# TobiaMarcucci/warm-start-hybrid-mpc

Hardware: AMD Instinct MI355X
Metric: QP subproblems/sec, cart-pole-with-walls N=20 synthetic frontier (higher is better)
Workload: dtype f64

## Files before the change

warm-start-hybrid-mpc_amd/csrc/hmpc_kernel.hip:

```cpp
#include <hip/hip_runtime.h>
#include <math.h>
#include <stdint.h>
#include <type_traits>

#include "hmpc_device.h"

#define WAVE 64
#define HMPC_REFINE_FROM_IT 12
#define HMPC_POLISH_RHO 1e5
#define HMPC_POLISH_RHO2 1e7
#define HMPC_POLISH_DELTA 1e-10
#define HMPC_RHO_OF(level) ((level) == 1 ? HMPC_POLISH_RHO2 : HMPC_POLISH_RHO)
#define HMPC_POLISH_ITERS 5
#define HMPC_POLISH_ROUNDS 6
#define HMPC_POLISH_ROUNDS_LAST 10
#define HMPC_ESC_MAX 2
#define HMPC_ESC_ITERS 6
#define HMPC_ESC_ENABLED(D) true
#define HMPC_LAM0_ROW 1
#ifndef HMPC_STABLE_DEN
#define HMPC_STABLE_DEN 1
#endif
#ifndef HMPC_PAIR
#define HMPC_PAIR 1
#endif
#ifndef HMPC_NARROW_PANEL
#define HMPC_NARROW_PANEL 1
#endif
#define HMPC_POLISH_ATTEMPTS 3
#define HMPC_RETRY (-1)
#define HMPC_POLISH_ROUNDS_WARM 3
#ifndef HMPC_POLISH_ROUNDS_OWN
#define HMPC_POLISH_ROUNDS_OWN 8
#endif
#define HMPC_POLISH_WARM_BMOVE 0.5
#define HMPC_POLISH_WARM_VMAX 1e-2
#ifndef HMPC_KERNEL_ATTR
#define HMPC_KERNEL_ATTR
#endif
#define DEV __device__ __forceinline__
#ifdef HMPC_NO_FENCE
#define HMPC_FENCE() do { } while (0)
#else
#define HMPC_FENCE() __builtin_amdgcn_sched_barrier(0)
#endif

#ifdef HMPC_STAMPS
#define DBG_SKIP(bit) (p.dbg & (1 << (bit)))
#define STAMP(k) do { long long now_ = clock64(); tacc[k] += now_ - tlast; tlast = clock64(); } while (0)
#define FSTAMP(k) do { long long now_ = clock64(); facc[k] += now_ - flast; flast = clock64(); } while (0)
#define FSTAMP_DECL long long flast = clock64()
static __device__ long long facc_dump[16];
#define FSTAMP_ARGS , long long *facc
#define FSTAMP_PASS , facc
#else
#define DBG_SKIP(bit) false
#define STAMP(k) do { } while (0)
#define FSTAMP(k) do { } while (0)
#define FSTAMP_DECL do { } while (0)
#define FSTAMP_ARGS
#define FSTAMP_PASS
#endif

DEV void lds_barrier()
{
    asm volatile("s_waitcnt lgkmcnt(0)\n\ts_barrier" ::: "memory");
}

DEV double wave_sum(double v)
{
#pragma unroll
    for (int o = 32; o > 0; o >>= 1) v += __shfl_xor(v, o);
    return v;
}
DEV double wave_max(double v)
{
#pragma unroll
    for (int o = 32; o > 0; o >>= 1) v = fmax(v, __shfl_xor(v, o));
    return v;
}
DEV double wave_min(double v)
{
#pragma unroll
    for (int o = 32; o > 0; o >>= 1) v = fmin(v, __shfl_xor(v, o));
    return v;
}

template <class D, int N>
DEV void block_reduce(double (&v)[N], const int (&op)[N], __attribute__((address_space(3))) double *red, int tid)
{
#pragma unroll
    for (int i = 0; i < N; i++) v[i] = op[i] == 0 ? wave_sum(v[i]) : op[i] == 1 ? wave_max(v[i]) : wave_min(v[i]);
    if constexpr (D::kNW > 1) {
        if ((tid & 63) == 0) {
#pragma unroll
            for (int i = 0; i < N; i++) red[(tid >> 6) * N + i] = v[i];
        }
        __syncthreads();
#pragma unroll
        for (int i = 0; i < N; i++) {
            double a = red[i];
#pragma unroll
            for (int w = 1; w < D::kNW; w++) {
                const double b = red[w * N + i];
                a = op[i] == 0 ? a + b : op[i] == 1 ? fmax(a, b) : fmin(a, b);
            }
            v[i] = a;
        }
        __syncthreads();
    }
}
template <class D> DEV double block_sum(double x, __attribute__((address_space(3))) double *red, int tid)
{
    double v[1] = {x};
    const int op[1] = {0};
    block_reduce<D, 1>(v, op, red, tid);
    return v[0];
}
template <class D> DEV double block_max(double x, __attribute__((address_space(3))) double *red, int tid)
{
    double v[1] = {x};
    const int op[1] = {1};
    block_reduce<D, 1>(v, op, red, tid);
    return v[0];
}
template <class D> DEV double block_min(double x, __attribute__((address_space(3))) double *red, int tid)
{
    double v[1] = {x};
    const int op[1] = {2};
    block_reduce<D, 1>(v, op, red, tid);
    return v[0];
}

DEV double bcast(double v, int src)
{
    const int lo = __builtin_amdgcn_readlane(__double2loint(v), src);
    const int hi = __builtin_amdgcn_readlane(__double2hiint(v), src);
    return __hiloint2double(hi, lo);
}

template <class D> DEV double bcast16(double v, int src)
{
    if constexpr (!D::kDpp) return bcast(v, src);
    const long x = __builtin_bit_cast(long, v);
    long r;
    switch (src) {
#define HMPC_DPP_CASE(n) case n: r = __builtin_amdgcn_update_dpp((long)0, x, 0x150 + n, 0xf, 0xf, false); break;
        HMPC_DPP_CASE(0) HMPC_DPP_CASE(1) HMPC_DPP_CASE(2) HMPC_DPP_CASE(3) HMPC_DPP_CASE(4) HMPC_DPP_CASE(5) HMPC_DPP_CASE(6) HMPC_DPP_CASE(7)
        HMPC_DPP_CASE(8) HMPC_DPP_CASE(9) HMPC_DPP_CASE(10) HMPC_DPP_CASE(11) HMPC_DPP_CASE(12) HMPC_DPP_CASE(13) HMPC_DPP_CASE(14)
#undef HMPC_DPP_CASE
    default: r = __builtin_amdgcn_update_dpp((long)0, x, 0x150 + 15, 0xf, 0xf, false); break;
    }
    return __builtin_bit_cast(double, r);
}

DEV double frcp(double b)
{
    double r = __builtin_amdgcn_rcp(b);
    r = fma(fma(-b, r, 1.0), r, r);
    r = fma(fma(-b, r, 1.0), r, r);
    return r;
}

typedef __attribute__((address_space(3))) double ldsd;
typedef __attribute__((address_space(3))) int ldsi;
typedef __attribute__((address_space(3))) unsigned char ldsb;

template <class IP, class DP>
struct Lists {
    IP rptr, rcol, cptr, crow, gptr, grow;
    DP rval, cval, gval, h;
};
typedef Lists<const ldsi *, const ldsd *> ListsL;
typedef Lists<const int *, const double *> ListsG;

struct Lds {
    ldsd *w, *lam, *nuf;
    ldsd *e;
    ldsd *Lm, *dinv, *Pr;
    ldsd *rd, *rdyn, *edyn, *g, *pv;
    ldsd *w1, *lam1, *nuf1, *w2, *lam2, *nuf2;
    ldsd *Mm, *PA, *q, *mv;
    ldsd *red;
    ldsi *flag;
    ldsd *x0;
    ldsi *fix;
    ldsd *AB, *P, *PT;
    ldsi *ei, *ej;
    ListsL L0;
    ListsG G0;
    double *LmG, *PrG;
    ldsd *Ls;
    ldsd *Lw;
    int abst, nup, lrows;
    const ldsd *Cdn, *sval;
    const ldsi *drow, *rinfo, *sptr, *srow, *nrow;
    const ldsd *ccv;
    const ldsb *cci;
    int term_on;
    unsigned long long fullfix;
};

template <int NX_, int NU_, int NUB_, int NW_, bool DPP_ = false>
struct Dims {
    static constexpr bool kDpp = DPP_;
    static constexpr int kNX = NX_, kNU = NU_, kNUB = NUB_;
    static constexpr int kNW = NW_, kNT = NW_ * 64;
    static constexpr bool kBig = NX_ < 0;
#ifdef HMPC_JIT_KC
    static constexpr int kKC = NX_ > 0 ? HMPC_JIT_KC : 0;
#else
    static constexpr int kKC = NX_ > 0 ? (NU_ == 7 ? 14 : 8) : 0;
#endif
    static DEV int nx(const DevProb &p) { return NX_ > 0 ? NX_ : p.nx; }
    static DEV int nu(const DevProb &p) { return NU_ > 0 ? NU_ : p.nu; }
    static DEV int nub(const DevProb &p) { return NU_ > 0 ? NUB_ : p.nub; }
    static DEV int nuc(const DevProb &p) { return NU_ > 0 ? NU_ - NUB_ : p.nuc; }
    static DEV int nz(const DevProb &p) { return NX_ > 0 ? NX_ + NU_ : p.nz; }
    static DEV int ne(const DevProb &p) { return NX_ > 0 ? (NX_ + NU_) * (NX_ + NU_ + 1) / 2 : p.ne; }
};

#define AB_STRIDE (D::kBig ? S.abst : nz)
template <class D> DEV decltype(auto) stage_lists(const Lds &S)
{
    if constexpr (D::kBig) return (S.G0);
    else return (S.L0);
}
template <class D> DEV auto fac_lm(const Lds &S)
{
    if constexpr (D::kBig) return S.LmG;
    else return S.Lm;
}
template <class D> DEV auto fac_pr(const Lds &S)
{
    if constexpr (D::kBig) return S.PrG;
    else return S.Pr;
}

template <int RS>
struct Rows {
    double s_[RS], zd_[RS], dz_[RS], prod_[RS];
    DEV double &s(int k, int) { return s_[k]; }
    DEV double &z(int k, int) { return zd_[k]; }
    DEV double &D(int k, int) { return zd_[k]; }
    DEV double &dz(int k, int) { return dz_[k]; }
    DEV double &prod(int k, int) { return prod_[k]; }
    DEV void bind(double *, int) {}
};
template <>
struct Rows<0> {
    double *__restrict__ s_, *__restrict__ zd_, *__restrict__ dz_, *__restrict__ prod_;
    DEV double &s(int, int r) { return s_[r]; }
    DEV double &z(int, int r) { return zd_[r]; }
    DEV double &D(int, int r) { return zd_[r]; }
    DEV double &dz(int, int r) { return dz_[r]; }
    DEV double &prod(int, int r) { return prod_[r]; }
    DEV void bind(double *base, int Mpad) { s_ = base; zd_ = base + Mpad; dz_ = base + 2 * Mpad; prod_ = base + 3 * Mpad; }
};
#define ROW_OPAQUE(r) asm volatile("" : "+v"(r))
#define LANE_OPAQUE(lane) asm volatile("" : "+v"(lane))
#ifdef HMPC_CHECK
#define HMPC_CHK(cond, bit) do { if (!(cond)) atomicOr(p.check_flag, 1u << (bit)); } while (0)
#else
#define HMPC_CHK(cond, bit) do { } while (0)
#endif
#define ROWS_BEGIN(k, rw)                                  \
    _Pragma("unroll") for (int k = 0; k < nslot; k++) {   \
        typename RM::Ref rw;                               \
        if (rm.at(p, k, lane, rw)) {                       \
            HMPC_CHK(rw.e >= 0 && rw.e < p.M, 0);
#define ROWS_END }}

DEV void row_decode(const DevProb &p, int r, int &t, int &lr)
{
    if (r >= p.Toff) {
        t = p.T - 1;
        lr = p.mreg + (r - p.Toff);
    } else {
        t = (int)__umulhi((unsigned)r, p.mreg_magic);
        lr = r - t * p.mreg;
    }
}

template <class D> DEV bool row_active(const DevProb &p, const ldsi *fix, int t, int lr, int term_on)
{
    const int nub = D::nub(p);
    if (lr >= p.mreg) return term_on;
    if (lr < p.nc) return true;
    int b = lr - p.nc;
    if (b >= nub) b -= nub;
    return fix[t * nub + b] < 0;
}

DEV int sym(int i, int l) { return i >= l ? i * (i + 1) / 2 + l : l * (l + 1) / 2 + i; }

template <class IP, class DP> DEV double list_dot(IP idx, DP val, int k0, int k1, const ldsd *v)
{
    double a0 = 0, a1 = 0, a2 = 0, a3 = 0;
    int k = k0;
    for (; k + 4 <= k1; k += 4) {
        const int i0 = idx[k], i1 = idx[k + 1], i2 = idx[k + 2], i3 = idx[k + 3];
        const double c0 = val[k], c1 = val[k + 1], c2 = val[k + 2], c3 = val[k + 3];
        a0 += c0 * v[i0];
        a1 += c1 * v[i1];
        a2 += c2 * v[i2];
        a3 += c3 * v[i3];
    }
    if (k + 2 <= k1) {
        const int i0 = idx[k], i1 = idx[k + 1];
        const double c0 = val[k], c1 = val[k + 1];
        a0 += c0 * v[i0];
        a1 += c1 * v[i1];
        k += 2;
    }
    if (k < k1) a2 += val[k] * v[idx[k]];
    return (a0 + a1) + (a2 + a3);
}
template <class L> DEV double row_dot(const L &st, int lr, const ldsd *v)
{
    return list_dot(st.rcol, st.rval, st.rptr[lr], st.rptr[lr + 1], v);
}
template <class L> DEV double col_dot(const L &st, int j, const ldsd *v)
{
    return list_dot(st.crow, st.cval, st.cptr[j], st.cptr[j + 1], v);
}
template <class L> DEV double gram(const L &st, int e, const ldsd *D)
{
    return list_dot(st.grow, st.gval, st.gptr[e], st.gptr[e + 1], D);
}
template <class D> DEV double crow_dot(const DevProb &p, const Lds &S, int lr, const ldsd *v)
{
    if constexpr (D::kBig) {
        if (S.Cdn && lr < p.mreg) {
            const int nz = D::nz(p);
            const int ri = S.rinfo[lr];
            if (ri >= 0) return S.sval[lr] * v[ri];
            const ldsd *c = S.Cdn + (-ri - 1) * nz;
            double a0 = 0, a1 = 0, a2 = 0, a3 = 0;
            int j = 0;
            for (; j + 4 <= nz; j += 4) {
                const double c0 = c[j], c1 = c[j + 1], c2 = c[j + 2], c3 = c[j + 3];
                const double v0 = v[j], v1 = v[j + 1], v2 = v[j + 2], v3 = v[j + 3];
                a0 += c0 * v0;
                a1 += c1 * v1;
                a2 += c2 * v2;
                a3 += c3 * v3;
            }
            for (; j < nz; j++) a0 += c[j] * v[j];
            return (a0 + a1) + (a2 + a3);
        }
    }
    if (lr < p.mreg) return row_dot(stage_lists<D>(S), lr, v);
    const int nz = D::nz(p);
    const double *c = p.Ct + (size_t)(lr - p.mreg) * nz;
    double a = 0;
    for (int j = 0; j < nz; j++) a += c[j] * v[j];
    return a;
}
template <class D> DEV double ccol_dot(const DevProb &p, const Lds &S, int t, int j, const ldsd *base)
{
    double a;
    if constexpr (D::kKC > 0) {
        const ldsd *eb = base + t * p.mreg, *cv = S.ccv + j * D::kKC;
        const ldsb *ci = S.cci + j * D::kKC;
        constexpr int H = D::kKC / 2;
        static_assert(D::kKC % 2 == 0, "padded columns come in two halves");
        double a0 = 0, a1 = 0;
#pragma unroll
        for (int hb = 0; hb < D::kKC; hb += H) {
            int idx[H];
            double cc[H], ee[H];
#pragma unroll
            for (int q = 0; q < H; q++) idx[q] = ci[hb + q];
#pragma unroll
            for (int q = 0; q < H; q++) cc[q] = cv[hb + q];
            HMPC_FENCE();
#pragma unroll
            for (int q = 0; q < H; q++) { HMPC_CHK(idx[q] >= 0 && idx[q] < p.mreg && j >= 0 && j < D::nz(p) && t >= 0 && t < p.T, 1); ee[q] = eb[idx[q]]; }
            HMPC_FENCE();
#pragma unroll
            for (int q = 0; q < H; q++) {
                if (q & 1) a1 += cc[q] * ee[q];
                else a0 += cc[q] * ee[q];
            }
        }
        a = a0 + a1;
    } else if (D::kBig && S.Cdn) {
        const int nz = D::nz(p);
        const ldsd *eb = base + t * p.mreg, *c = S.Cdn + j;
        double a0 = 0, a1 = 0;
        int r = 0;
        for (; r + 2 <= p.nd; r += 2) {
            a0 += c[r * nz] * eb[S.drow[r]];
            a1 += c[(r + 1) * nz] * eb[S.drow[r + 1]];
        }
        if (r < p.nd) a0 += c[r * nz] * eb[S.drow[r]];
        for (int k = S.sptr[j]; k < S.sptr[j + 1]; k++) {
            const int sr = S.srow[k];
            a1 += S.sval[sr] * eb[sr];
        }
        a = a0 + a1;
    } else {
        a = col_dot(stage_lists<D>(S), j, base + t * p.mreg);
    }
    if (S.term_on && t == p.T - 1) {
        if constexpr (D::kKC > 0) {
            a += S.mv[j];
        } else {
            const int nz = D::nz(p);
            const ldsd *vt = base + p.Toff;
            double a0 = 0, a1 = 0;
            int k = 0;
            for (; k + 2 <= p.nT; k += 2) {
                a0 += p.Ct[(size_t)k * nz + j] * vt[k];
                a1 += p.Ct[(size_t)(k + 1) * nz + j] * vt[k + 1];
            }
            if (k < p.nT) a0 += p.Ct[(size_t)k * nz + j] * vt[k];
            a += a0 + a1;
        }
    }
    return a;
}

template <class D, class RM> DEV void term_cols(const DevProb &p, const Lds &S, int lane, const ldsd *base)
{
    if constexpr (D::kKC > 0) {
        if (!S.term_on) return;
        constexpr int NZ = D::kNX + D::kNU, KT = RM::kSlots - RM::kSlotsFB;
        double acc[NZ];
#pragma unroll
        for (int j = 0; j < NZ; j++) acc[j] = 0.0;
#pragma unroll
        for (int k = 0; k < KT; k++) {
            const int row = k * D::kNT + lane;
            const bool ok = row < p.nT;
            const int rc = ok ? row : 0;
            const double v = ok ? base[p.Toff + rc] : 0.0;
            const double *c = p.Ct + (size_t)rc * NZ;
#pragma unroll
            for (int j = 0; j < NZ; j++) acc[j] += c[j] * v;
        }
        if constexpr (D::kNW == 1) {
#pragma unroll
            for (int j = 0; j < NZ; j++) acc[j] = wave_sum(acc[j]);
        } else {
            constexpr int CH = 40 / D::kNW;
#pragma unroll
            for (int j0 = 0; j0 < NZ; j0 += CH) {
                double v[CH];
                int op[CH];
#pragma unroll
                for (int q = 0; q < CH; q++) { v[q] = j0 + q < NZ ? acc[j0 + q] : 0.0; op[q] = 0; }
                block_reduce<D, CH>(v, op, S.red, lane);
#pragma unroll
// ... 1368 lines not shown
        for (int i = lane; i < nx; i += D::kNT) dw[i] = usex0 ? S.x0[i] : 0.0;
        __syncthreads();
    }
    for (int t = wave_sweeps ? T : 0; t < T; t++) {
        const auto Lm = fac_lm<D>(S) + t * lms;
        const ldsi *fx = S.fix + t * nub;
        const ldsd *x = dw + t * nz;
        for (int j = lane; j < nu; j += D::kNT) {
            double a = S.dinv[t * nu + j] * dw[t * nz + nx + j];
            const bool fixed = j >= nuc && fx[j - nuc] >= 0;
            if (!fixed)
                for (int l = 0; l < nx; l++) a += Lm[LM_X(nx, nu, l, j)] * x[l];
            S.mv[j] = a;
        }
        __syncthreads();
        for (int j = nu - 1; j >= 1; j--) {
            const double uj = S.mv[j];
            for (int i = lane; i < j; i += D::kNT) {
                const bool fixed = i >= nuc && fx[i - nuc] >= 0;
                if (!fixed) S.mv[i] -= Lm[LM_U(nx, nu, j, i)] * uj;
            }
            __syncthreads();
        }
        for (int i = lane; i < nu; i += D::kNT) dw[t * nz + nx + i] = -S.mv[i];
        __syncthreads();
        for (int i = lane; i < nx; i += D::kNT) {
            double a = csrc ? cs * csrc[t * nx + i] : 0.0;
            for (int l = 0; l < nz; l++) a += S.AB[i * AB_STRIDE + l] * dw[t * nz + l];
            dw[(t + 1) * nz + i] = a;
        }
        __syncthreads();
    }
    for (int o = lane; o < (T + 1) * nx; o += D::kNT) {
        const int t = o / nx, i = o - t * nx;
        double a = S.pv[o];
        const auto Pt = fac_pr<D>(S) + t * nxs;
        int l = 0;
        for (; l + 4 <= nx; l += 4) {
            const double p0 = Pt[sym(i, l)], p1 = Pt[sym(i, l + 1)], p2 = Pt[sym(i, l + 2)], p3 = Pt[sym(i, l + 3)];
            a += p0 * dw[t * nz + l] + p1 * dw[t * nz + l + 1] + p2 * dw[t * nz + l + 2] + p3 * dw[t * nz + l + 3];
        }
        for (; l < nx; l++) a += Pt[sym(i, l)] * dw[t * nz + l];
        dlam[o] = -a;
    }
    FSTAMP(8);
    {
        const int nslot = RS > 0 ? RS : p.Mpad / D::kNT;
        ROWS_BEGIN(k, rw)
            const double d = R.D(k, rw.e);
            if (d != 0.0)
                S.e[rw.e] = d * rm.dot(p, S, k, rw, dw) - S.e[rw.e];
        ROWS_END
    }
    __syncthreads();
    FSTAMP(9);
    const bool own_g = gsrc && gsrc != S.g;
    for (int o = lane; o < T * nub; o += D::kNT) {
        const int t = o / nub, b = o - t * nub;
        double a = 0;
        if (S.fix[o] >= 0) {
            const int c = nx + nuc + b;
            a = own_g ? gs * gsrc[t * nz + c] : 0.0;
            for (int j = 0; j < nz; j++) a -= S.P[c * nz + j] * dw[t * nz + j];
            a -= ccol_dot<D>(p, S, t, c, S.e);
            for (int l = 0; l < nx; l++) a += S.AB[l * AB_STRIDE + c] * dlam[(t + 1) * nx + l];
        }
        dnuf[o] = a;
    }
    for (int i = lane; i < nx; i += D::kNT) {
        double a = own_g ? gs * gsrc[i] : 0.0;
        for (int j = 0; j < nz; j++) a -= S.P[i * nz + j] * dw[j];
        a -= ccol_dot<D>(p, S, 0, i, S.e);
        for (int l = 0; l < nx; l++) a += S.AB[l * AB_STRIDE + i] * dlam[nx + l];
        dlam[i] = a;
    }
    __syncthreads();
    FSTAMP(10);
}

template <class D, int RS, class RM>
DEV void kkt_solve_reg(const DevProb &p, const Lds &S, Rows<RS> &R, const RM &rm, int lane, const ldsd *gsrc, double gs, bool usex0,
                       const ldsd *csrc, double cs, bool useb, ldsd *dw, ldsd *dlam, ldsd *dnuf FSTAMP_ARGS)
{
    constexpr int NX = D::kNX, NU = D::kNU, NUB = D::kNUB, NUC = NU - NUB, NZ = NX + NU;
    constexpr int NXS = NX * (NX + 1) / 2, LMS = LM_STAGE(NX, NU);
    const int T = p.T;
    FSTAMP_DECL;
    LANE_OPAQUE(lane);
    term_cols<D, RM>(p, S, lane, S.e);
    for (int o = lane; o < T * NZ; o += D::kNT) {
        const int t = o / NZ, j = o - t * NZ;
        const double a = (gsrc ? gs * gsrc[o] : 0.0) + ccol_dot<D>(p, S, t, j, S.e);
        S.g[o] = (useb ? S.g[o] : 0.0) - a;
    }
    for (int o = lane; o < T * NX; o += D::kNT) {
        const int t = o / NX, i = o - t * NX;
        double a = 0.0;
        if (csrc) {
#pragma unroll
            for (int l = 0; l < NX; l++) a += S.Pr[(t + 1) * NXS + sym(i, l)] * (cs * csrc[t * NX + l]);
        }
        S.pv[o] = a;
    }
    double pvr = 0.0;
    if (lane < NX) {
        pvr = -(gsrc ? gs * gsrc[T * NZ + lane] : 0.0);
        S.pv[T * NX + lane] = pvr;
    }
    __syncthreads();
    FSTAMP(6);
    LANE_OPAQUE(lane);
    if (D::kNW == 1 || lane < WAVE) {
        double ABcol[NX];
#pragma unroll
        for (int l = 0; l < NX; l++) ABcol[l] = lane < NZ ? S.AB[l * NZ + lane] : 0.0;
        const int rowoff = lane < NX ? lane * NU : lane < NZ ? LM_U(NX, NU, lane - NX, 0) : 0;
        const int rowlen = lane < NX ? NU : lane < NZ ? lane - NX : 0;
        const int gl = lane < NZ ? lane : 0, bl = (lane >= NX + NUC && lane < NZ) ? lane - NX - NUC : 0;
        const int pl = lane < NX ? lane : 0;
        double mrow_n[NU], mpre_n, qc_n;
        int f_n;
        {
            const ldsd *row = S.Lm + (T - 1) * LMS + rowoff;
#pragma unroll
            for (int j = 0; j < NU; j++) mrow_n[j] = row[j];
            mpre_n = S.g[(T - 1) * NZ + gl];
            f_n = S.fix[(T - 1) * NUB + bl];
            qc_n = S.pv[(T - 1) * NX + pl];
        }
        for (int t = T - 1; t >= 0; t--) {
            double mrow[NU];
#pragma unroll
            for (int j = 0; j < NU; j++) mrow[j] = j < rowlen ? mrow_n[j] : 0.0;
            const double mpre = lane < NZ ? mpre_n : 0.0;
            const int f = (lane >= NX + NUC && lane < NZ) ? f_n : -1;
            const double qv = pvr + qc_n;
            {
                const int tn = t > 0 ? t - 1 : 0;
                const ldsd *row = S.Lm + tn * LMS + rowoff;
#pragma unroll
                for (int j = 0; j < NU; j++) mrow_n[j] = row[j];
                mpre_n = S.g[tn * NZ + gl];
                f_n = S.fix[tn * NUB + bl];
                qc_n = S.pv[tn * NX + pl];
            }
            double v = mpre;
#pragma unroll
            for (int l = 0; l < NX; l++) v += ABcol[l] * bcast16<D>(qv, l);
            if (f >= 0) v = (useb && f == 1) ? -1.0 : 0.0;
#pragma unroll
            for (int j = 0; j < NUC; j++) v -= mrow[j] * bcast16<D>(v, NX + j);
            if (!((S.fullfix >> t) & 1ull)) {
#pragma unroll
                for (int j = NUC; j < NU; j++) v -= mrow[j] * bcast16<D>(v, NX + j);
            }
            if (lane >= NX && lane < NZ) dw[t * NZ + lane] = v;
            pvr = v;
            if (lane < NX) S.pv[t * NX + lane] = v;
        }
    }
    __syncthreads();
    FSTAMP(7);
    LANE_OPAQUE(lane);
    if (D::kNW == 1 || lane < WAVE) {
        double ABrow[NZ];
#pragma unroll
        for (int l = 0; l < NZ; l++) ABrow[l] = lane < NX ? S.AB[lane * NZ + l] : 0.0;
        double xr = (lane < NX && usex0) ? S.x0[lane] : 0.0;
        const int cl = lane < NU ? lane : 0, pl = lane < NX ? lane : 0;
        double lx_n[NX], lcol_n[NU], dinv_n, y_n, cdy_n;
        {
            const ldsd *colp = S.Lm + cl;
#pragma unroll
            for (int l = 0; l < NX; l++) lx_n[l] = colp[LM_X(NX, NU, l, 0)];
#pragma unroll
            for (int i = 1; i < NU; i++) lcol_n[i] = colp[LM_U(NX, NU, i, 0)];
            dinv_n = S.dinv[cl];
            y_n = dw[NX + cl];
            cdy_n = csrc ? csrc[pl] : 0.0;
        }
        for (int t = 0; t < T; t++) {
            double lx[NX], lcol[NU];
#pragma unroll
            for (int l = 0; l < NX; l++) lx[l] = lane < NU ? lx_n[l] : 0.0;
            lcol[0] = 0.0;
#pragma unroll
            for (int i = 1; i < NU; i++) lcol[i] = lane < i ? lcol_n[i] : 0.0;
            double cur = lane < NU ? dinv_n * y_n : 0.0;
            double xn = (csrc && lane < NX) ? cs * cdy_n : 0.0;
            {
                const int tn = t + 1 < T ? t + 1 : t;
                const ldsd *colp = S.Lm + tn * LMS + cl;
#pragma unroll
                for (int l = 0; l < NX; l++) lx_n[l] = colp[LM_X(NX, NU, l, 0)];
#pragma unroll
                for (int i = 1; i < NU; i++) lcol_n[i] = colp[LM_U(NX, NU, i, 0)];
                dinv_n = S.dinv[tn * NU + cl];
                y_n = dw[tn * NZ + NX + cl];
                cdy_n = csrc ? csrc[tn * NX + pl] : 0.0;
            }
#pragma unroll
            for (int l = 0; l < NX; l++) {
                const double xl = bcast16<D>(xr, l);
                cur += lx[l] * xl;
                xn += ABrow[l] * xl;
            }
#pragma unroll
            for (int j = NU - 1; j >= 0; j--) {
                const double uj = bcast16<D>(cur, j);
                cur -= lcol[j] * uj;
                xn -= ABrow[NX + j] * uj;
            }
            if (lane < NX) dw[t * NZ + lane] = xr;
            if (lane < NU) dw[t * NZ + NX + lane] = -cur;
            xr = xn;
        }
        if (lane < NX) dw[T * NZ + lane] = xr;
    }
    __syncthreads();
    FSTAMP(9);
    LANE_OPAQUE(lane);
    for (int o = lane; o < (T + 1) * NX; o += D::kNT) {
        const int t = o / NX, i = o - t * NX;
        double a = S.pv[o];
#pragma unroll
        for (int l = 0; l < NX; l++) a += S.Pr[t * NXS + sym(i, l)] * dw[t * NZ + l];
        dlam[o] = -a;
    }
    if constexpr (!D::kDpp) {
        const int nslot = RS;
        ROWS_BEGIN(k, rw)
            const double d = R.D(k, rw.e);
            if (d != 0.0)
                S.e[rw.e] = d * rm.dot(p, S, k, rw, dw) - S.e[rw.e];
        ROWS_END
    } else {
        constexpr int KS = RM::kSlotsFB;
        double val[KS];
#pragma unroll
        for (int k = 0; k < KS; k++) {
            typename RM::Ref rw;
            const bool ok = rm.at(p, k, lane, rw);
            const double d = ok ? R.D(k, rw.e) : 0.0;
            val[k] = d * rm.dot_all(k, ok, rw, dw) - S.e[ok ? rw.e : 0];
            if (d == 0.0) val[k] = __longlong_as_double(0x7ff8000000000000LL);
        }
#pragma unroll
        for (int k = 0; k < KS; k++) {
            typename RM::Ref rw;
            (void)rm.at(p, k, lane, rw);
            if (val[k] == val[k]) S.e[rw.e] = val[k];
        }
        if (S.term_on) {
#pragma unroll
            for (int k = KS; k < RS; k++) {
                typename RM::Ref rw;
                if (rm.at(p, k, lane, rw)) {
                    const double d = R.D(k, rw.e);
                    if (d != 0.0) S.e[rw.e] = d * rm.dot(p, S, k, rw, dw) - S.e[rw.e];
                }
            }
        }
    }
    __syncthreads();
    const bool own_g = gsrc && gsrc != S.g;
    term_cols<D, RM>(p, S, lane, S.e);
    for (int o = lane; o < T * NUB; o += D::kNT) {
        const int t = o / NUB, b = o - t * NUB;
        double a = 0;
        if (S.fix[o] >= 0) {
            const int c = NX + NUC + b;
            a = own_g ? gs * gsrc[t * NZ + c] : 0.0;
#pragma unroll
            for (int j = 0; j < NZ; j++) a -= S.P[c * NZ + j] * dw[t * NZ + j];
            a -= ccol_dot<D>(p, S, t, c, S.e);
#pragma unroll
            for (int l = 0; l < NX; l++) a += S.AB[l * NZ + c] * dlam[(t + 1) * NX + l];
        }
        dnuf[o] = a;
    }
    if constexpr (HMPC_LAM0_ROW) {
        if (lane < NX) {
            double a = own_g ? gs * gsrc[lane] : 0.0;
#pragma unroll
            for (int j = 0; j < NZ; j++) a -= S.P[lane * NZ + j] * dw[j];
            a -= ccol_dot<D>(p, S, 0, lane, S.e);
#pragma unroll
            for (int l = 0; l < NX; l++) a += S.AB[l * NZ + lane] * dlam[NX + l];
            dlam[lane] = a;
        }
    }
    __syncthreads();
    FSTAMP(10);
}

template <class D, int RS, class RM>
DEV double kkt_solve_reg_pair(const DevProb &p, const Lds &S, Rows<RS> &R, const RM &rm, int lane, double tau FSTAMP_ARGS)
{
    constexpr int NX = D::kNX, NU = D::kNU, NUB = D::kNUB, NUC = NU - NUB, NZ = NX + NU;
    constexpr int NXS = NX * (NX + 1) / 2, LMS = LM_STAGE(NX, NU);
    const int T = p.T;
    const int nslot = RS;
    ldsd *pv2 = S.edyn;
    FSTAMP_DECL;
    LANE_OPAQUE(lane);
    ROWS_BEGIN(k, rw)
        S.e[rw.e] = R.D(k, rw.e) * rm.h(p, S, k, rw);
    ROWS_END
    __syncthreads();
    term_cols<D, RM>(p, S, lane, S.e);
    for (int o = lane; o < T * NZ; o += D::kNT) {
        const int t = o / NZ, j = o - t * NZ;
        S.g[o] = S.g[o] - ccol_dot<D>(p, S, t, j, S.e);
    }
    for (int o = lane; o < (T + 1) * NX; o += D::kNT) S.pv[o] = 0.0;
    __syncthreads();
    ROWS_BEGIN(k, rw)
        double v = 0;
        const double d = R.D(k, rw.e);
        if (d != 0.0) {
            const double sr = R.s(k, rw.e), zr = d * sr;
            const double rc = sr - rm.h(p, S, k, rw) * tau + rm.dot(p, S, k, rw, S.w);
            const double dsr = sr * zr;
            v = dsr * frcp(sr) - 1.0 * (d * rc);
        }
        S.e[rw.e] = v;
        R.dz(k, rw.e) = v;
    ROWS_END
    __syncthreads();
    term_cols<D, RM>(p, S, lane, S.e);
    for (int o = lane; o < T * NZ; o += D::kNT) {
        const int t = o / NZ, j = o - t * NZ;
        const double a = -1.0 * S.rd[o] + ccol_dot<D>(p, S, t, j, S.e);
        S.w2[o] = 0.0 - a;
    }
    for (int o = lane; o < T * NX; o += D::kNT) {
        const int t = o / NX, i = o - t * NX;
        double a = 0.0;
#pragma unroll
        for (int l = 0; l < NX; l++) a += S.Pr[(t + 1) * NXS + sym(i, l)] * (-1.0 * S.rdyn[t * NX + l]);
        pv2[o] = a;
    }
    double pvrA = 0.0, pvrB = 0.0;
    if (lane < NX) {
        pvrB = -(-1.0 * S.rd[T * NZ + lane]);
        pv2[T * NX + lane] = pvrB;
    }
    __syncthreads();
    FSTAMP(6);
    LANE_OPAQUE(lane);
    if (D::kNW == 1 || lane < WAVE) {
        double ABcol[NX];
#pragma unroll
        for (int l = 0; l < NX; l++) ABcol[l] = lane < NZ ? S.AB[l * NZ + lane] : 0.0;
        const int rowoff = lane < NX ? lane * NU : lane < NZ ? LM_U(NX, NU, lane - NX, 0) : 0;
        const int rowlen = lane < NX ? NU : lane < NZ ? lane - NX : 0;
        const int gl = lane < NZ ? lane : 0, bl = (lane >= NX + NUC && lane < NZ) ? lane - NX - NUC : 0;
        const int pl = lane < NX ? lane : 0;
        double mrow_n[NU], mpreA_n, mpreB_n, qcA_n, qcB_n;
        int f_n;
        {
            const ldsd *row = S.Lm + (T - 1) * LMS + rowoff;
#pragma unroll
            for (int j = 0; j < NU; j++) mrow_n[j] = row[j];
            mpreA_n = S.g[(T - 1) * NZ + gl];
            mpreB_n = S.w2[(T - 1) * NZ + gl];
            f_n = S.fix[(T - 1) * NUB + bl];
            qcA_n = S.pv[(T - 1) * NX + pl];
            qcB_n = pv2[(T - 1) * NX + pl];
        }
        for (int t = T - 1; t >= 0; t--) {
            double mrow[NU];
#pragma unroll
            for (int j = 0; j < NU; j++) mrow[j] = j < rowlen ? mrow_n[j] : 0.0;
            const double mpreA = lane < NZ ? mpreA_n : 0.0, mpreB = lane < NZ ? mpreB_n : 0.0;
            const int f = (lane >= NX + NUC && lane < NZ) ? f_n : -1;
            const double qvA = pvrA + qcA_n, qvB = pvrB + qcB_n;
            {
                const int tn = t > 0 ? t - 1 : 0;
                const ldsd *row = S.Lm + tn * LMS + rowoff;
#pragma unroll
                for (int j = 0; j < NU; j++) mrow_n[j] = row[j];
                mpreA_n = S.g[tn * NZ + gl];
                mpreB_n = S.w2[tn * NZ + gl];
                f_n = S.fix[tn * NUB + bl];
                qcA_n = S.pv[tn * NX + pl];
                qcB_n = pv2[tn * NX + pl];
            }
            double vA = mpreA, vB = mpreB;
#pragma unroll
            for (int l = 0; l < NX; l++) {
                vA += ABcol[l] * bcast16<D>(qvA, l);
                vB += ABcol[l] * bcast16<D>(qvB, l);
            }
            if (f >= 0) { vA = (f == 1) ? -1.0 : 0.0; vB = 0.0; }
#pragma unroll
            for (int j = 0; j < NUC; j++) {
                vA -= mrow[j] * bcast16<D>(vA, NX + j);
                vB -= mrow[j] * bcast16<D>(vB, NX + j);
            }
            if (!((S.fullfix >> t) & 1ull)) {
#pragma unroll
                for (int j = NUC; j < NU; j++) {
                    vA -= mrow[j] * bcast16<D>(vA, NX + j);
                    vB -= mrow[j] * bcast16<D>(vB, NX + j);
                }
            }
            if (lane >= NX && lane < NZ) { S.w1[t * NZ + lane] = vA; S.w2[t * NZ + lane] = vB; }
            pvrA = vA;
            pvrB = vB;
            if (lane < NX) { S.pv[t * NX + lane] = vA; pv2[t * NX + lane] = vB; }
        }
    }
    __syncthreads();
    FSTAMP(7);
    LANE_OPAQUE(lane);
    if (D::kNW == 1 || lane < WAVE) {
        double ABrow[NZ];
#pragma unroll
        for (int l = 0; l < NZ; l++) ABrow[l] = lane < NX ? S.AB[lane * NZ + l] : 0.0;
        double xrA = lane < NX ? S.x0[lane] : 0.0, xrB = 0.0;
        const int cl = lane < NU ? lane : 0, pl = lane < NX ? lane : 0;
        double lx_n[NX], lcol_n[NU], dinv_n, yA_n, yB_n, cdy_n;
        {
            const ldsd *colp = S.Lm + cl;
#pragma unroll
            for (int l = 0; l < NX; l++) lx_n[l] = colp[LM_X(NX, NU, l, 0)];
#pragma unroll
            for (int i = 1; i < NU; i++) lcol_n[i] = colp[LM_U(NX, NU, i, 0)];
            dinv_n = S.dinv[cl];
            yA_n = S.w1[NX + cl];
            yB_n = S.w2[NX + cl];
            cdy_n = S.rdyn[pl];
        }
        for (int t = 0; t < T; t++) {
            double lx[NX], lcol[NU];
#pragma unroll
            for (int l = 0; l < NX; l++) lx[l] = lane < NU ? lx_n[l] : 0.0;
            lcol[0] = 0.0;
#pragma unroll
            for (int i = 1; i < NU; i++) lcol[i] = lane < i ? lcol_n[i] : 0.0;
            double curA = lane < NU ? dinv_n * yA_n : 0.0, curB = lane < NU ? dinv_n * yB_n : 0.0;
            double xnA = 0.0, xnB = lane < NX ? -1.0 * cdy_n : 0.0;
            {
                const int tn = t + 1 < T ? t + 1 : t;
                const ldsd *colp = S.Lm + tn * LMS + cl;
#pragma unroll
                for (int l = 0; l < NX; l++) lx_n[l] = colp[LM_X(NX, NU, l, 0)];
#pragma unroll
                for (int i = 1; i < NU; i++) lcol_n[i] = colp[LM_U(NX, NU, i, 0)];
                dinv_n = S.dinv[tn * NU + cl];
                yA_n = S.w1[tn * NZ + NX + cl];
                yB_n = S.w2[tn * NZ + NX + cl];
                cdy_n = S.rdyn[tn * NX + pl];
            }
#pragma unroll
            for (int l = 0; l < NX; l++) {
                const double xlA = bcast16<D>(xrA, l), xlB = bcast16<D>(xrB, l);
                curA += lx[l] * xlA;
                curB += lx[l] * xlB;
                xnA += ABrow[l] * xlA;
                xnB += ABrow[l] * xlB;
            }
#pragma unroll
            for (int j = NU - 1; j >= 0; j--) {
                const double ujA = bcast16<D>(curA, j), ujB = bcast16<D>(curB, j);
                curA -= lcol[j] * ujA;
                curB -= lcol[j] * ujB;
                xnA -= ABrow[NX + j] * ujA;
                xnB -= ABrow[NX + j] * ujB;
            }
            if (lane < NX) { S.w1[t * NZ + lane] = xrA; S.w2[t * NZ + lane] = xrB; }
            if (lane < NU) { S.w1[t * NZ + NX + lane] = -curA; S.w2[t * NZ + NX + lane] = -curB; }
            xrA = xnA;
            xrB = xnB;
        }
        if (lane < NX) { S.w1[T * NZ + lane] = xrA; S.w2[T * NZ + lane] = xrB; }
    }
    __syncthreads();
    FSTAMP(9);
    LANE_OPAQUE(lane);
    for (int o = lane; o < (T + 1) * NX; o += D::kNT) {
        const int t = o / NX, i = o - t * NX;
        double a = S.pv[o], b = pv2[o];
#pragma unroll
        for (int l = 0; l < NX; l++) {
            const double pr = S.Pr[t * NXS + sym(i, l)];
            a += pr * S.w1[t * NZ + l];
            b += pr * S.w2[t * NZ + l];
        }
        S.lam1[o] = -a;
        S.lam2[o] = -b;
    }
    double q2 = 0.0;
    ROWS_BEGIN(k, rw)
        const double d = R.D(k, rw.e);
        double z1 = 0.0;
        if (d != 0.0) {
            z1 = d * rm.dot(p, S, k, rw, S.w1) - d * rm.h(p, S, k, rw);
            q2 += z1 * z1 * frcp(d);
        }
        S.e[rw.e] = z1;
    ROWS_END
    __syncthreads();
    term_cols<D, RM>(p, S, lane, S.e);
    for (int o = lane; o < T * NUB; o += D::kNT) {
        const int t = o / NUB, b = o - t * NUB;
        double a = 0;
        if (S.fix[o] >= 0) {
            const int c = NX + NUC + b;
#pragma unroll
            for (int j = 0; j < NZ; j++) a -= S.P[c * NZ + j] * S.w1[t * NZ + j];
            a -= ccol_dot<D>(p, S, t, c, S.e);
#pragma unroll
            for (int l = 0; l < NX; l++) a += S.AB[l * NZ + c] * S.lam1[(t + 1) * NX + l];
        }
        S.nuf1[o] = a;
    }
    if (lane < NX) {
        double a = 0.0;
#pragma unroll
        for (int j = 0; j < NZ; j++) a -= S.P[lane * NZ + j] * S.w1[j];
        a -= ccol_dot<D>(p, S, 0, lane, S.e);
#pragma unroll
        for (int l = 0; l < NX; l++) a += S.AB[l * NZ + lane] * S.lam1[NX + l];
        S.lam1[lane] = a;
    }
    __syncthreads();
    ROWS_BEGIN(k, rw)
        const double d = R.D(k, rw.e);
        double z2 = 0.0;
        if (d != 0.0) z2 = d * rm.dot(p, S, k, rw, S.w2) - R.dz(k, rw.e);
        S.e[rw.e] = z2;
    ROWS_END
    __syncthreads();
    term_cols<D, RM>(p, S, lane, S.e);
    for (int o = lane; o < T * NUB; o += D::kNT) {
        const int t = o / NUB, b = o - t * NUB;
        double a = 0;
        if (S.fix[o] >= 0) {
            const int c = NX + NUC + b;
            a = -1.0 * S.rd[t * NZ + c];
#pragma unroll
            for (int j = 0; j < NZ; j++) a -= S.P[c * NZ + j] * S.w2[t * NZ + j];
            a -= ccol_dot<D>(p, S, t, c, S.e);
#pragma unroll
            for (int l = 0; l < NX; l++) a += S.AB[l * NZ + c] * S.lam2[(t + 1) * NX + l];
        }
        S.nuf2[o] = a;
    }
    if (lane < NX) {
        double a = -1.0 * S.rd[lane];
#pragma unroll
        for (int j = 0; j < NZ; j++) a -= S.P[lane * NZ + j] * S.w2[j];
        a -= ccol_dot<D>(p, S, 0, lane, S.e);
#pragma unroll
        for (int l = 0; l < NX; l++) a += S.AB[l * NZ + lane] * S.lam2[NX + l];
        S.lam2[lane] = a;
    }
    __syncthreads();
    FSTAMP(10);
    return q2;
}

template <class D, int RS, class RM>
DEV void kkt_dispatch(const DevProb &p, const Lds &S, Rows<RS> &R, const RM &rm, int lane, const ldsd *gsrc, double gs, bool usex0,
                      const ldsd *csrc, double cs, bool useb, ldsd *dw, ldsd *dlam, ldsd *dnuf FSTAMP_ARGS)
{
    if constexpr (D::kNX > 0) kkt_solve_reg<D, RS>(p, S, R, rm, lane, gsrc, gs, usex0, csrc, cs, useb, dw, dlam, dnuf FSTAMP_PASS);
    else kkt_solve<D, RS>(p, S, R, rm, lane, gsrc, gs, usex0, csrc, cs, useb, dw, dlam, dnuf FSTAMP_PASS);
}

template <class D, class RM>
DEV double lin_obj(const DevProb &p, const Lds &S, const RM &rm, int lane, const ldsd *lam, const ldsd *nuf, const ldsd *zrow)
{
    double a = 0;
    LANE_OPAQUE(lane);
    for (int j = lane; j < D::nx(p); j += D::kNT) a += S.x0[j] * lam[j];
    for (int o = lane; o < p.T * D::nub(p); o += D::kNT)
        if (S.fix[o] == 1) a += nuf[o];
    const int nslot = RM::kSlots > 0 ? RM::kSlots : p.Mpad / D::kNT;
    ROWS_BEGIN(k, rw)
        if (rm.active(p, S, k, rw)) a += rm.h(p, S, k, rw) * zrow[rw.e];
    ROWS_END
    return a;
}

template <class D> DEV void set_prescribed(const DevProb &p, const Lds &S, int lane, double tau)
{
    const int nub = D::nub(p);
    for (int i = lane; i < D::nx(p); i += D::kNT) S.w[i] = S.x0[i] * tau;
    for (int o = lane; o < p.T * nub; o += D::kNT)
        if (S.fix[o] >= 0) S.w[(o / nub) * D::nz(p) + D::nx(p) + D::nuc(p) + (o % nub)] = S.fix[o] * tau;
}

template <class D> DEV double wPv(const DevProb &p, const Lds &S, int lane, const ldsd *v)
{
    const int nx = D::nx(p), nz = D::nz(p), T = p.T, n = T * nz + nx;
    double acc = 0;
    LANE_OPAQUE(lane);
    for (int o = lane; o < n; o += D::kNT) {
        const int t = o / nz < T ? o / nz : T;
        const int i = o - t * nz, dim = t < T ? nz : nx;
        const ldsd *PP = t < T ? S.P : S.PT;
        double a = 0;
        for (int j = 0; j < dim; j++) a += PP[i * dim + j] * v[t * nz + j];
        acc += a * S.w[o];
    }
    return acc;
}

template <class D> DEV double dPd(const DevProb &p, const Lds &S, int lane, const ldsd *v, double sc)
{
    const int nx = D::nx(p), nz = D::nz(p), T = p.T, n = T * nz + nx;
    double acc = 0;
    LANE_OPAQUE(lane);
    for (int o = lane; o < n; o += D::kNT) {
        const int t = o / nz < T ? o / nz : T;
        const int i = o - t * nz, dim = t < T ? nz : nx;
        const ldsd *PP = t < T ? S.P : S.PT;
        double a = 0;
        for (int j = 0; j < dim; j++) a += PP[i * dim + j] * (sc * S.w[t * nz + j] - v[t * nz + j]);
        acc += a * (sc * S.w[o] - v[o]);
    }
    return acc;
}

template <class D, int RS, class RM, bool WARM>
DEV int ipm_solve(const DevProb &p, const Lds &S, Rows<RS> &R, RM &rm, int lane, int term_on, int &iters, double &tau_out,
                  bool &polished_out, int &weak_out, bool &handed_out, double *trace, const double *wprim, const double *wdual,
                  bool attempt_only, bool own = false)
{
    const int nx = D::nx(p), nz = D::nz(p), T = p.T, nuc = D::nuc(p), nub = D::nub(p), M = p.M, n = T * nz + nx;
    const int nslot = RS > 0 ? RS : p.Mpad / D::kNT;
    int mact = 0;
    rm.prepare(p, S, lane, term_on);
    ROWS_BEGIN(k, rw)
        const bool on = rm.active(p, S, k, rw);
        mact += on;
        R.s(k, rw.e) = 1.0;
        R.z(k, rw.e) = on ? 1.0 : 0.0;
    ROWS_END
    mact = (int)block_sum<D>((double)mact, S.red, lane);
    for (int i = lane; i < n; i += D::kNT) S.w[i] = 0.0;
    for (int i = lane; i < (T + 1) * nx; i += D::kNT) S.lam[i] = 0.0;
    for (int i = lane; i < T * nub; i += D::kNT) S.nuf[i] = 0.0;
    double tau = 1.0, kap = 1.0;
    __syncthreads();
    set_prescribed<D>(p, S, lane, tau);
    __syncthreads();
    double x0inf = 0;
    for (int i = lane; i < nx; i += D::kNT) x0inf = fmax(x0inf, fabs(S.x0[i]));
    x0inf = block_max<D>(x0inf, S.red, lane);

    int status = HMPC_MAXITER, it = 0, extra_done = 0;
    polished_out = false;
    weak_out = 0;
    handed_out = false;
    bool tried = false;
    int attempts = 0;
    double last_alpha = 0, last_dtau = 0, last_dkap = 0;
#ifdef HMPC_TRACE_STEP
    double dbg_den = 0;
#endif
#ifdef HMPC_STAMPS
    long long tacc[8] = {0, 0, 0, 0, 0, 0, 0, 0}, tlast = clock64();
    long long facc[16] = {0, 0, 0, 0, 0, 0, 0, 0, 0, 0, 0, 0, 0, 0, 0, 0};
#endif
    int mode = 0, round = 0, al = 0;
    int level = p.polish_l1;
    double rg = 0, mu = 0, wPw = 0, winf = 0, zinf = 0;
    bool warm_try = false;
    if constexpr (WARM) if (wprim != nullptr && p.polish) {
        const int nu = D::nu(p);
        for (int o = lane; o < n; o += D::kNT) {
            const int t = o / nz < T ? o / nz : T;
            const int j = o - t * nz;
            S.w[o] = j < nx ? wprim[t * nx + j] : wprim[(T + 1) * nx + t * nu + (j - nx)];
        }
        __syncthreads();
        double bmove = 0.0;
        for (int o = lane; o < T * nub; o += D::kNT)
            if (S.fix[o] >= 0) bmove = fmax(bmove, fabs(S.w[(o / nub) * nz + nx + nuc + (o % nub)] - (double)S.fix[o]));
        bmove = block_max<D>(bmove, S.red, lane);
        set_prescribed<D>(p, S, lane, 1.0);
        __syncthreads();
        const int o_mu = (T + 1) * nx, o_lb = o_mu + (T - 1) * p.nc + p.ncL, o_ub = o_lb + T * nub;
        double wi = 0, zi = 0;
        for (int o = lane; o < n; o += D::kNT) wi = fmax(wi, fabs(S.w[o]));
        for (int o = lane; o < (T + 1) * nx; o += D::kNT) zi = fmax(zi, fabs(wdual[o]) * p.cs);
        ROWS_BEGIN(k, rw)
            double d = 0.0;
            if (rm.active(p, S, k, rw)) {
                int t, lr;
                row_decode(p, rw.e, t, lr);
                double zr;
                if (lr < p.nc) zr = wdual[o_mu + t * p.nc + lr] * p.cs / p.reg.scale[lr];
                else if (lr >= p.mreg) zr = wdual[o_mu + t * p.nc + p.nc + (lr - p.mreg)] * p.cs / p.sct[lr - p.mreg];
                else if (lr < p.nc + nub) zr = wdual[o_lb + t * nub + (lr - p.nc)] * p.cs;
                else zr = wdual[o_ub + t * nub + (lr - p.nc - nub)] * p.cs;
                zi = fmax(zi, zr);
                R.prod(k, rw.e) = 1.0;
                if (zr > 0.0) { d = HMPC_RHO_OF(p.polish_l1); R.dz(k, rw.e) = zr; }
                else { d = HMPC_POLISH_DELTA; R.dz(k, rw.e) = rm.dot(p, S, k, rw, S.w); }
                R.D(k, rw.e) = d;
            }
            S.e[rw.e] = d;
        ROWS_END
        {
            double v[2] = {wi, zi};
            const int op[2] = {1, 1};
            block_reduce<D, 2>(v, op, S.red, lane);
            winf = v[0]; zinf = v[1];
        }
        if (winf == winf && zinf == zinf && bmove <= HMPC_POLISH_WARM_BMOVE) { mode = 1; warm_try = true; }
        else {
            ROWS_BEGIN(k, rw)
                if (R.D(k, rw.e) != 0.0) R.z(k, rw.e) = 1.0;
            ROWS_END
            for (int o = lane; o < n; o += D::kNT) S.w[o] = 0.0;
            __syncthreads();
            set_prescribed<D>(p, S, lane, tau);
        }
        __syncthreads();
        if (attempt_only && !warm_try) {
            iters = 0;
            tau_out = tau;
            return HMPC_RETRY;
        }
    }
    for (it = 0; it <= p.max_iter;) {
      if (mode == 0) {
        STAMP(7);
        LANE_OPAQUE(lane);
        ROWS_BEGIN(k, rw)
            S.e[rw.e] = R.z(k, rw.e);
        ROWS_END
        __syncthreads();
        wPw = 0;
        for (int o = lane; o < n; o += D::kNT) {
            const int t = o / nz < T ? o / nz : T;
            const int i = o - t * nz, dim = t < T ? nz : nx;
            const ldsd *PP = t < T ? S.P : S.PT;
            double a = 0;
            for (int j = 0; j < dim; j++) a += PP[i * dim + j] * S.w[t * nz + j];
            wPw += a * S.w[o];
        }
        double rdinf = 0, certinf = 0, fy = 0, yinf = 0;
        winf = 0;
        term_cols<D, RM>(p, S, lane, S.e);
        for (int o = lane; o < n; o += D::kNT) {
            const int t = o / nz < T ? o / nz : T;
            const int j = o - t * nz;
            double a = 0;
            if (t == T) {
                a = S.lam[T * nx + j];
            } else {
                if (j < nx) a += S.lam[t * nx + j];
                for (int l = 0; l < nx; l++) a -= S.AB[l * AB_STRIDE + j] * S.lam[(t + 1) * nx + l];
                if (j >= nx + nuc && S.fix[t * nub + (j - nx - nuc)] >= 0) a += S.nuf[t * nub + (j - nx - nuc)];
                a += ccol_dot<D>(p, S, t, j, S.e);
            }
            double pw = 0;
            {
                const int dim = t < T ? nz : nx;
                const ldsd *PP = t < T ? S.P : S.PT;
                for (int l = 0; l < dim; l++) pw += PP[j * dim + l] * S.w[t * nz + l];
            }
            const double v = pw + a;
            S.rd[o] = v;
            rdinf = fmax(rdinf, fabs(v));
            certinf = fmax(certinf, fabs(a));
            winf = fmax(winf, fabs(S.w[o]));
        }
        double rcinf = 0;
        for (int o = lane; o < T * nx; o += D::kNT) {
            const int t = o / nx, i = o - t * nx;
            double a = S.w[(t + 1) * nz + i];
            for (int l = 0; l < nz; l++) a -= S.AB[i * AB_STRIDE + l] * S.w[t * nz + l];
            S.rdyn[o] = a;
// ... 1044 lines not shown
```

Before: 631,800.

## Pack paired KKT right-hand sides into separate DPP rows of one wave

Adds a packed mode, now the default through HMPC_PAIR=2, for the paired backward and forward Riccati sweeps in kkt_solve_reg_pair. Each of the two right-hand sides now uses its own 16-lane row, and broadcasts use row-wise DPP, so every step does one chain of broadcasts and FMAs instead of two interleaved ones. This cuts the instruction count on the serial recurrence. In exchange, lanes in rows 2 and 3 do idle work, and the packed path only applies to single-wave configurations.

```diff
diff --git a/warm-start-hybrid-mpc_amd/csrc/hmpc_kernel.hip b/warm-start-hybrid-mpc_amd/csrc/hmpc_kernel.hip
--- a/warm-start-hybrid-mpc_amd/csrc/hmpc_kernel.hip
+++ b/warm-start-hybrid-mpc_amd/csrc/hmpc_kernel.hip
@@ -22,7 +22,7 @@
 #define HMPC_STABLE_DEN 1
 #endif
 #ifndef HMPC_PAIR
-#define HMPC_PAIR 1
+#define HMPC_PAIR 2
 #endif
 #ifndef HMPC_NARROW_PANEL
 #define HMPC_NARROW_PANEL 1
@@ -150,6 +150,20 @@
         HMPC_DPP_CASE(8) HMPC_DPP_CASE(9) HMPC_DPP_CASE(10) HMPC_DPP_CASE(11) HMPC_DPP_CASE(12) HMPC_DPP_CASE(13) HMPC_DPP_CASE(14)
 #undef HMPC_DPP_CASE
     default: r = __builtin_amdgcn_update_dpp((long)0, x, 0x150 + 15, 0xf, 0xf, false); break;
+    }
+    return __builtin_bit_cast(double, r);
+}
+
+DEV double bcast_rows(double v, int src)
+{
+    const long x = __builtin_bit_cast(long, v);
+    long r;
+    switch (src) {
+#define HMPC_DPP_CASE(n) case n: r = __builtin_amdgcn_update_dpp((long)0, x, 0x150 + n, 0xf, 0xf, true); break;
+        HMPC_DPP_CASE(0) HMPC_DPP_CASE(1) HMPC_DPP_CASE(2) HMPC_DPP_CASE(3) HMPC_DPP_CASE(4) HMPC_DPP_CASE(5) HMPC_DPP_CASE(6) HMPC_DPP_CASE(7)
+        HMPC_DPP_CASE(8) HMPC_DPP_CASE(9) HMPC_DPP_CASE(10) HMPC_DPP_CASE(11) HMPC_DPP_CASE(12) HMPC_DPP_CASE(13) HMPC_DPP_CASE(14)
+#undef HMPC_DPP_CASE
+    default: r = __builtin_amdgcn_update_dpp((long)0, x, 0x150 + 15, 0xf, 0xf, true); break;
     }
     return __builtin_bit_cast(double, r);
 }
@@ -2124,6 +2138,7 @@
     const int T = p.T;
     const int nslot = RS;
     ldsd *pv2 = S.edyn;
+    constexpr bool kPacked = HMPC_PAIR == 2 && D::kNW == 1;
     FSTAMP_DECL;
     LANE_OPAQUE(lane);
     ROWS_BEGIN(k, rw)
@@ -2163,7 +2178,7 @@
         for (int l = 0; l < NX; l++) a += S.Pr[(t + 1) * NXS + sym(i, l)] * (-1.0 * S.rdyn[t * NX + l]);
         pv2[o] = a;
     }
-    double pvrA = 0.0, pvrB = 0.0;
+    [[maybe_unused]] double pvrA = 0.0, pvrB = 0.0;
     if (lane < NX) {
         pvrB = -(-1.0 * S.rd[T * NZ + lane]);
         pv2[T * NX + lane] = pvrB;
@@ -2171,6 +2186,63 @@
     __syncthreads();
     FSTAMP(6);
     LANE_OPAQUE(lane);
+    if constexpr (kPacked) {
+    if (D::kNW == 1 || lane < WAVE) {
+        const int r = lane >> 4, c = lane & 15;
+        const bool on = r < 2, rowB = r == 1;
+        double ABcol[NX];
+#pragma unroll
+        for (int l = 0; l < NX; l++) ABcol[l] = c < NZ ? S.AB[l * NZ + c] : 0.0;
+        const int rowoff = c < NX ? c * NU : c < NZ ? LM_U(NX, NU, c - NX, 0) : 0;
+        const int rowlen = c < NX ? NU : c < NZ ? c - NX : 0;
+        const int gl = c < NZ ? c : 0, bl = (c >= NX + NUC && c < NZ) ? c - NX - NUC : 0;
+        const int pl = c < NX ? c : 0;
+        const ldsd *gsrc = rowB ? S.w2 : S.g;
+        ldsd *pdst = rowB ? pv2 : S.pv, *ydst = rowB ? S.w2 : S.w1;
+        double pvr = 0.0;
+        if (rowB && c < NX) pvr = pv2[T * NX + c];
+        double mrow_n[NU], mpre_n, qc_n;
+        int f_n;
+        {
+            const ldsd *row = S.Lm + (T - 1) * LMS + rowoff;
+#pragma unroll
+            for (int j = 0; j < NU; j++) mrow_n[j] = row[j];
+            mpre_n = gsrc[(T - 1) * NZ + gl];
+            f_n = S.fix[(T - 1) * NUB + bl];
+            qc_n = pdst[(T - 1) * NX + pl];
+        }
+        for (int t = T - 1; t >= 0; t--) {
+            double mrow[NU];
+#pragma unroll
+            for (int j = 0; j < NU; j++) mrow[j] = j < rowlen ? mrow_n[j] : 0.0;
+            const double mpre = (on && c < NZ) ? mpre_n : 0.0;
+            const int f = (c >= NX + NUC && c < NZ) ? f_n : -1;
+            const double qv = pvr + (on ? qc_n : 0.0);
+            {
+                const int tn = t > 0 ? t - 1 : 0;
+                const ldsd *row = S.Lm + tn * LMS + rowoff;
+#pragma unroll
+                for (int j = 0; j < NU; j++) mrow_n[j] = row[j];
+                mpre_n = gsrc[tn * NZ + gl];
+                f_n = S.fix[tn * NUB + bl];
+                qc_n = pdst[tn * NX + pl];
+            }
+            double v = mpre;
+#pragma unroll
+            for (int l = 0; l < NX; l++) v += ABcol[l] * bcast_rows(qv, l);
+            if (f >= 0) v = (r == 0 && f == 1) ? -1.0 : 0.0;
+#pragma unroll
+            for (int j = 0; j < NUC; j++) v -= mrow[j] * bcast_rows(v, NX + j);
+            if (!((S.fullfix >> t) & 1ull)) {
+#pragma unroll
+                for (int j = NUC; j < NU; j++) v -= mrow[j] * bcast_rows(v, NX + j);
+            }
+            if (on && c >= NX && c < NZ) ydst[t * NZ + c] = v;
+            pvr = v;
+            if (on && c < NX) pdst[t * NX + c] = v;
+        }
+    }
+    } else {
     if (D::kNW == 1 || lane < WAVE) {
         double ABcol[NX];
 #pragma unroll
@@ -2234,9 +2306,70 @@
             if (lane < NX) { S.pv[t * NX + lane] = vA; pv2[t * NX + lane] = vB; }
         }
     }
+    }
     __syncthreads();
     FSTAMP(7);
     LANE_OPAQUE(lane);
+    if constexpr (kPacked) {
+    if (D::kNW == 1 || lane < WAVE) {
+        const int r = lane >> 4, c = lane & 15;
+        const bool on = r < 2, rowB = r == 1;
+        double ABrow[NZ];
+#pragma unroll
+        for (int l = 0; l < NZ; l++) ABrow[l] = c < NX ? S.AB[c * NZ + l] : 0.0;
+        double xr = (r == 0 && c < NX) ? S.x0[c] : 0.0;
+        const int cl = c < NU ? c : 0, pl = c < NX ? c : 0;
+        ldsd *dw = rowB ? S.w2 : S.w1;
+        double lx_n[NX], lcol_n[NU], dinv_n, y_n, cdy_n;
+        {
+            const ldsd *colp = S.Lm + cl;
+#pragma unroll
+            for (int l = 0; l < NX; l++) lx_n[l] = colp[LM_X(NX, NU, l, 0)];
+#pragma unroll
+            for (int i = 1; i < NU; i++) lcol_n[i] = colp[LM_U(NX, NU, i, 0)];
+            dinv_n = S.dinv[cl];
+            y_n = dw[NX + cl];
+            cdy_n = S.rdyn[pl];
+        }
+        for (int t = 0; t < T; t++) {
+            double lx[NX], lcol[NU];
+#pragma unroll
+            for (int l = 0; l < NX; l++) lx[l] = c < NU ? lx_n[l] : 0.0;
+            lcol[0] = 0.0;
+#pragma unroll
+            for (int i = 1; i < NU; i++) lcol[i] = c < i ? lcol_n[i] : 0.0;
+            double cur = (on && c < NU) ? dinv_n * y_n : 0.0;
+            double xn = (rowB && c < NX) ? -1.0 * cdy_n : 0.0;
+            {
+                const int tn = t + 1 < T ? t + 1 : t;
+                const ldsd *colp = S.Lm + tn * LMS + cl;
+#pragma unroll
+                for (int l = 0; l < NX; l++) lx_n[l] = colp[LM_X(NX, NU, l, 0)];
+#pragma unroll
+                for (int i = 1; i < NU; i++) lcol_n[i] = colp[LM_U(NX, NU, i, 0)];
+                dinv_n = S.dinv[tn * NU + cl];
+                y_n = dw[tn * NZ + NX + cl];
+                cdy_n = S.rdyn[tn * NX + pl];
+            }
+#pragma unroll
+            for (int l = 0; l < NX; l++) {
+                const double xl = bcast_rows(xr, l);
+                cur += lx[l] * xl;
+                xn += ABrow[l] * xl;
+            }
+#pragma unroll
+            for (int j = NU - 1; j >= 0; j--) {
+                const double uj = bcast_rows(cur, j);
+                cur -= lcol[j] * uj;
+                xn -= ABrow[NX + j] * uj;
+            }
+            if (on && c < NX) dw[t * NZ + c] = xr;
+            if (on && c < NU) dw[t * NZ + NX + c] = -cur;
+            xr = xn;
+        }
+        if (on && c < NX) dw[T * NZ + c] = xr;
+    }
+    } else {
     if (D::kNW == 1 || lane < WAVE) {
         double ABrow[NZ];
 #pragma unroll
@@ -2298,6 +2431,7 @@
             xrB = xnB;
         }
         if (lane < NX) { S.w1[T * NZ + lane] = xrA; S.w2[T * NZ + lane] = xrB; }
+    }
     }
     __syncthreads();
     FSTAMP(9);
```

New measurement: 554,000. 12.3% lower.
